# drocheam/optrace

Measured on AMD Instinct MI355X. Metric: ray-surface-intersections/s, higher is better.
Workload: dtype f64

## Files before the change

optrace_amd/csrc/ot_api.hip:

```cpp
#include <cstdlib>
#include <cstring>
#include <string>

#include "ot_host.hpp"
#include "ot_selftest.hpp"

static thread_local std::string g_err;

int fail(int code, const std::string& msg) {
    g_err = msg;
    return code;
}

extern "C" int ot_abi_version(void) { return OT_ABI_VERSION; }
extern "C" const char* ot_last_error(void) { return g_err.c_str(); }
extern "C" int ot_device_count(void) {
    int n = 0;
    if (hipGetDeviceCount(&n) != hipSuccess) return OT_ERR_NO_DEVICE;
    return n;
}

int require_device() {
    int n = 0;
    if (hipGetDeviceCount(&n) != hipSuccess || n <= 0)
        return fail(OT_ERR_NO_DEVICE, "no HIP device available; this library has no CPU fallback");
    return OT_OK;
}

static void* ws_alloc(size_t bytes) {
    void* p = nullptr;
    if (hipMalloc(&p, bytes) != hipSuccess || !p) {
        (void)hipGetLastError();
        return nullptr;
    }
    return p;
}
static void ws_release(void* p) { (void)hipFree(p); }
static void ws_sync() { (void)hipDeviceSynchronize(); }
static ot_scratch::Pool& scratch_pool() {
    static ot_scratch::Pool pool({ws_alloc, ws_release, ws_sync}, [] {
        const char* v = std::getenv("OT_SCRATCH_CAP_GB");
        const double gb = v ? std::atof(v) : 64.0;
        return (size_t)((gb > 0.0 ? gb : 64.0) * 1e9);
    }());
    return pool;
}

ot_scratch::Lease workspace(int purpose, size_t bytes, hipStream_t st) {
    int dev = 0;
    if (hipGetDevice(&dev) != hipSuccess) return {};
    return ot_scratch::Lease(scratch_pool(), dev, purpose, (void*)st, bytes);
}

extern "C" int ot_scratch_trim(void) {
    if (int rc = require_device()) return rc;
    scratch_pool().trim();
    return OT_OK;
}

extern "C" int ot_scratch_set_cap(int64_t bytes) {
    if (bytes < 0) return fail(OT_ERR_INVALID, "ot_scratch_set_cap: negative cap");
    scratch_pool().set_cap((size_t)bytes);
    return OT_OK;
}

extern "C" int ot_scratch_stats(int64_t* kept_bytes, int32_t* blocks, int32_t* leased) {
    size_t kept = 0;
    int nb = 0, busy = 0;
    scratch_pool().stats(&kept, &nb, &busy);
    if (kept_bytes) *kept_bytes = (int64_t)kept;
    if (blocks) *blocks = nb;
    if (leased) *leased = busy;
    return OT_OK;
}

int cu_count() {
    int dev = 0;
    hipDeviceProp_t prop;
    if (hipGetDevice(&dev) == hipSuccess && hipGetDeviceProperties(&prop, dev) == hipSuccess && prop.multiProcessorCount > 0)
        return prop.multiProcessorCount;
    return 256;
}

extern "C" int ot_selftest_arith(int32_t op, int32_t operand_class, int64_t n, uint64_t seed, int64_t* mismatches,
                                 double* first_bad4, void* stream) {
    if (!mismatches || !first_bad4 || n < 0) return fail(OT_ERR_INVALID, "ot_selftest_arith: bad argument");
    if (op < OT_ST_DIV || op > OT_ST_DIV_SHARED || operand_class < OT_CLS_WIDE || operand_class > OT_CLS_COSINE)
        return fail(OT_ERR_INVALID, "ot_selftest_arith: unknown operation or operand class");
    if (int rc = require_device()) return rc;
    hipStream_t st = (hipStream_t)stream;
    char* scratch = nullptr;
    HIP_TRY(hipMalloc((void**)&scratch, 64));
    hipError_t e = hipMemsetAsync(scratch, 0, 64, st);
    unsigned long long host[2] = {0, 0};
    double bad[4] = {0, 0, 0, 0};
    if (e == hipSuccess && n > 0) {
        hipLaunchKernelGGL(selftest_arith_kernel, dim3((unsigned)(cu_count() * 8)), dim3(256), 0, st, (int)op,
                           (int)operand_class, n, seed, (unsigned long long*)scratch, (double*)(scratch + 16));
        e = hipGetLastError();
    }
    if (e == hipSuccess) e = hipMemcpyAsync(host, scratch, 16, hipMemcpyDeviceToHost, st);
    if (e == hipSuccess) e = hipMemcpyAsync(bad, scratch + 16, 32, hipMemcpyDeviceToHost, st);
    if (e == hipSuccess) e = hipStreamSynchronize(st);
    (void)hipFree(scratch);
    HIP_TRY(e);
    *mismatches = (int64_t)host[0];
    std::memcpy(first_bad4, bad, sizeof(bad));
    return OT_OK;
}

extern "C" int ot_selftest_eval(int32_t op, int64_t n, const double* a, const double* b, const double* c, double* core_out,
                                double* ieee_out, void* stream) {
    if (n < 0 || (n && (!a || !core_out || !ieee_out))) return fail(OT_ERR_INVALID, "ot_selftest_eval: bad argument");
    if (op < OT_ST_DIV || op > OT_ST_DIV_SHARED) return fail(OT_ERR_INVALID, "ot_selftest_eval: unknown operation");
    if (int rc = require_device()) return rc;
    if (n == 0) return OT_OK;
    hipLaunchKernelGGL(selftest_eval_kernel, grid_for(n), dim3(256), 0, (hipStream_t)stream, (int)op, n, a, b, c, core_out,
                       ieee_out);
    HIP_TRY(hipGetLastError());
    return OT_OK;
}
```

optrace_amd/csrc/ot_device.hpp:

```cpp
#pragma once
#include <hip/hip_runtime.h>
#include <math.h>

#include "ot_scene.hpp"

#define OT_DEV __device__ __forceinline__
#define OT_HD __host__ __device__ __forceinline__

#define OT_CONST __attribute__((address_space(4)))
template <class T>
OT_DEV const OT_CONST T* as_const(const T* p) {
    return (const OT_CONST T*)p;
}

struct V3 {
    double x, y, z;
};

OT_DEV double dot3(const V3& a, const V3& b) { return a.x * b.x + a.y * b.y + a.z * b.z; }

OT_DEV V3 cross3(const V3& a, const V3& b) {
    V3 n;
    n.x = a.y * b.z - a.z * b.y;
    n.y = a.z * b.x - a.x * b.z;
    n.z = a.x * b.y - a.y * b.x;
    return n;
}

OT_DEV double ot_sqrt(double x) {
    double y = __builtin_amdgcn_rsq(x);
    double g = x * y;
    double h = 0.5 * y;
    double r = __builtin_fma(-h, g, 0.5);
    g = __builtin_fma(g, r, g);
    h = __builtin_fma(h, r, h);
    double d = __builtin_fma(-g, g, x);
    g = __builtin_fma(d, h, g);
    d = __builtin_fma(-g, g, x);
    g = __builtin_fma(d, h, g);
    return (x == 0.0 || x == __builtin_inf()) ? x : g;
}

OT_DEV double ot_rcp3(double d) {
    double r = __builtin_amdgcn_rcp(d);
    r = __builtin_fma(__builtin_fma(-d, r, 1.0), r, r);
    return __builtin_fma(__builtin_fma(-d, r, 1.0), r, r);
}

OT_DEV double ot_div_r(double n, double d, double r) {
    double q = n * r;
    return __builtin_fma(__builtin_fma(-d, q, n), r, q);
}

OT_DEV double ot_rsqrt(double x) {
    double y = __builtin_amdgcn_rsq(x);
    double e = __builtin_fma(-(x * y), y, 1.0);
    y = __builtin_fma(0.5 * y, e, y);
    e = __builtin_fma(-(x * y), y, 1.0);
    return __builtin_fma(0.5 * y, e, y);
}

OT_DEV V3 normalize3(const V3& a) {
    const double l = ot_sqrt(a.x * a.x + a.y * a.y + a.z * a.z);
    const double il = ot_rcp3(l);
    V3 r = {ot_div_r(a.x, l, il), ot_div_r(a.y, l, il), ot_div_r(a.z, l, il)};
    return r;
}

OT_HD double ot_div(double n, double d) {
#if defined(__HIP_DEVICE_COMPILE__)
    return ot_div_r(n, d, ot_rcp3(d));
#else
    return n / d;
#endif
}

OT_DEV V3 along(const V3& p, const V3& s, double t) {
    V3 r = {p.x + s.x * t, p.y + s.y * t, p.z + s.z * t};
    return r;
}

#include "ot_spline.hpp"

#define OT_HIT_CLOSED 0
#define OT_HIT_ILLINOIS 1
#define OT_HIT_SPLINE 2

template <class SF>
OT_HD double data_values_rel(SF& sf, double x, double y, PatchCache* pc = nullptr) {
    const double* t = sf.tab;
    const int n = sf.nk;
    double v;
    const UniformKnots ukv = {sf.ku_t0, sf.ku_h, sf.ku_inv_h, sf.ku_lo, sf.ku_hi,
                              (sf.ku_h > 0.0) ? OT_SPL_K + 1 : (1 << 30), n - OT_SPL_K - 2};
    const UniformKnots* const uk = &ukv;
    if (sf.kind == OT_SURF_DATA1D) {
        v = spl1_eval<OT_SPL_K>(t, n, t + n, sf.inv_h, hypot(x, y), uk, pc);
    } else {
        double xr = x, yr = y;
        if (sf.rot) {
            xr = x * sf.cna - y * sf.sna;
            yr = x * sf.sna + y * sf.cna;
        }
        v = spl2_eval<OT_SPL_K, OT_SPL_K>(t, n, t, n, t + n, sf.inv_h, xr, sf.sgn * yr, pc, uk);
    }
    return sf.sgn * (v - sf.offs);
}

template <class SF>
OT_HD void data_gradient(SF& sf, double x, double y, double& gx, double& gy, PatchCache* pc = nullptr) {
    const double* t = sf.tab;
    const int n = sf.nk;
    const UniformKnots ukv = {sf.ku_t0, sf.ku_h, sf.ku_inv_h, sf.ku_lo, sf.ku_hi,
                              (sf.ku_h > 0.0) ? OT_SPL_K + 1 : (1 << 30), n - OT_SPL_K - 2};
    const UniformKnots* const uk = &ukv;
    if (sf.kind == OT_SURF_DATA1D) {
        const double r = hypot(x, y);
        double d1;
        if (!spl1_grad_cached(t + n, r, uk, pc, d1)) d1 = spl1_eval<OT_SPL_K - 1>(t, n, t + 2 * n, sf.inv_h, r, uk);
        const double nr = sf.sgn * d1;
        const double rr = sqrt(x * x + y * y);
        gx = nr * ((rr > 0.0) ? x / rr : 1.0);
        gy = nr * ((rr > 0.0) ? y / rr : 0.0);
        return;
    }
    double xr = x, yr = y;
    if (sf.rot && !sf.deriv_unrot) {
        xr = x * sf.cna - y * sf.sna;
        yr = x * sf.sna + y * sf.cna;
    }
    const int nc = (n - OT_SPL_K - 1), ncx = (n - OT_SPL_K - 2) * nc;
    const double* c = t + n;
    double nxn, nyn;
    if (spl2_grad_cached(t, n, c, sf.inv_h, xr, sf.sgn * yr, pc, nxn, nyn, uk)) {
        nxn = nxn * sf.sgn;
    } else {
        nxn = spl2_eval<OT_SPL_K - 1, OT_SPL_K>(t + 1, n - 2, t, n, c + nc * nc, sf.inv_h, xr, sf.sgn * yr) * sf.sgn;
        nyn = spl2_eval<OT_SPL_K, OT_SPL_K - 1>(t, n, t + 1, n - 2, c + nc * nc + ncx, sf.inv_h, xr, sf.sgn * yr);
    }
    if (sf.rot) {
        gx = nxn * sf.cpa - nyn * sf.spa;
        gy = nxn * sf.spa + nyn * sf.cpa;
    } else {
        gx = nxn;
        gy = nyn;
    }
}

template <class SF>
OT_HD bool mask_table(SF& sf, double dx, double dy) {
    const uint32_t* words = (const uint32_t*)(sf.tab + sf.mask_off);
    const int n = sf.mask_n;
    int64_t cell;
    if (sf.kind == OT_SURF_DATA1D) {
        const int i = (int)(sqrt(dx * dx + dy * dy) * sf.mask_scale);
        cell = i < n ? i : n - 1;
    } else {
        double xr = dx, yr = dy;
        if (sf.rot) {
            xr = dx * sf.cna - dy * sf.sna;
            yr = dx * sf.sna + dy * sf.cna;
        }
        yr = sf.sgn * yr;
        int ix = (int)floor((xr + sf.mask_r) * sf.mask_scale), iy = (int)floor((yr + sf.mask_r) * sf.mask_scale);
        ix = ix < 0 ? 0 : (ix < n ? ix : n - 1);
        iy = iy < 0 ? 0 : (iy < n ? iy : n - 1);
        cell = (int64_t)iy * n + ix;
    }
    return (words[cell >> 5] >> (uint32_t)(cell & 31)) & 1u;
}

template <bool TABLES = true, class SF>
OT_DEV bool surf_mask(SF& sf, double x, double y) {
    if (sf.kind == OT_SURF_RECT || sf.kind == OT_SURF_SLIT) {
        double dx = x - sf.px, dy = y - sf.py;
        double xr = dx, yr = dy;
        if (sf.rot) {
            xr = dx * sf.cna - dy * sf.sna;
            yr = dx * sf.sna + dy * sf.cna;
        }
        bool outer = (sf.ox_lo <= xr) && (xr <= sf.ox_hi) && (sf.oy_lo <= yr) && (yr <= sf.oy_hi);
        if (sf.kind == OT_SURF_RECT) return outer;
        bool inner = (sf.ix_lo <= xr) && (xr <= sf.ix_hi) && (sf.iy_lo <= yr) && (yr <= sf.iy_hi);
        return outer && !inner;
    }
    double dx = x - sf.px, dy = y - sf.py;
    double r2 = dx * dx + dy * dy;
    bool in = r2 <= sf.r_eps2;
    if (sf.kind == OT_SURF_RING) in = in && (sf.ri_eps2 <= r2);
    if (TABLES && (sf.kind == OT_SURF_DATA1D || sf.kind == OT_SURF_DATA2D) && sf.mask_n) {
        if (in) in = mask_table(sf, dx, dy);
    }
    return in;
}

template <class SF>
OT_DEV double asph_poly(SF& sf, double r) {
    double y = 0.0;
    for (int j = sf.ncoeff - 1; j >= 0; j--) {
        y = y * r + sf.coeff[j];
        y = y * r + 0.0;
    }
    y = y * r + 0.0;
    return y;
}

template <class SF>
OT_DEV double asph_poly_deriv(SF& sf, double r) {
    double y = 0.0;
    for (int j = sf.ncoeff - 1; j >= 0; j--) {
        y = y * r + sf.dcoeff[j];
        y = y * r + 0.0;
    }
    return y;
}

#define OT_ASPH_CHUNK 4
OT_HD int asph_padded(int ncoeff) { return (ncoeff + OT_ASPH_CHUNK - 1) / OT_ASPH_CHUNK * OT_ASPH_CHUNK; }

template <bool DERIV, class SF>
OT_DEV double asph_poly_long(SF& sf, double r) {
    const int npad = asph_padded(sf.ncoeff);
    const OT_CONST double* c = (const OT_CONST double*)sf.tab + (DERIV ? npad : 0);
    double y = 0.0;
#pragma unroll 1
    for (int j = npad - OT_ASPH_CHUNK; j >= 0; j -= OT_ASPH_CHUNK) {
        const double c0 = c[j], c1 = c[j + 1], c2 = c[j + 2], c3 = c[j + 3];
        y = (y * r + c3) * r;
        y = (y * r + c2) * r;
        y = (y * r + c1) * r;
        y = (y * r + c0) * r;
    }
    return y;
}

template <int LEVEL = OT_HIT_SPLINE, class SF>
OT_DEV double surf_values_rel(SF& sf, double x, double y, PatchCache* pc = nullptr) {
    if (sf.kind == OT_SURF_TILTED) return x * sf.mx + y * sf.my;
    if (LEVEL >= OT_HIT_SPLINE && (sf.kind == OT_SURF_DATA1D || sf.kind == OT_SURF_DATA2D)) return data_values_rel(sf, x, y, pc);
    if (sf.kind == OT_SURF_CONIC) {
        double r2 = x * x + y * y;
        return ot_div(sf.rho * r2, 1 + sqrt(1 - sf.k1rho2 * r2));
    }
    double r = sqrt(x * x + y * y);
    double rr = r * r;
    double z = ot_div(sf.rho * rr, 1 + sqrt(1 - sf.k1rho2 * rr));
    if (LEVEL >= OT_HIT_SPLINE && sf.ncoeff > OT_MAX_ASPH)
        z += asph_poly_long<false>(sf, r) * r;
    else
        z += asph_poly(sf, r);
    return z;
}

template <int LEVEL = OT_HIT_SPLINE, class SF>
OT_DEV double surf_values(SF& sf, double x, double y, PatchCache* pc = nullptr) {
    if (sf.flat) return sf.z_max;
    if (surf_mask<(LEVEL >= OT_HIT_SPLINE)>(sf, x, y)) return sf.pz + surf_values_rel<LEVEL>(sf, x - sf.px, y - sf.py, pc);
    if (sf.kind == OT_SURF_TILTED || (LEVEL >= OT_HIT_SPLINE && sf.kind == OT_SURF_DATA2D)) {
        double dx = x - sf.px, dy = y - sf.py;
        double rr = sqrt(dx * dx + dy * dy);
        double c = (rr > 0.0) ? dx / rr : 1.0, sn = (rr > 0.0) ? dy / rr : 0.0;
        return sf.pz + surf_values_rel<LEVEL>(sf, sf.r_edge * c, sf.r_edge * sn, pc);
    }
    return sf.edge_val;
}

template <bool INSIDE = false, int LEVEL = OT_HIT_SPLINE, class SF>
OT_DEV V3 surf_normal(SF& sf, double x, double y, PatchCache* pc = nullptr) {
    constexpr bool TABLES = LEVEL >= OT_HIT_SPLINE;
    V3 n = {0.0, 0.0, 1.0};
    if (sf.kind < OT_SURF_CONIC) return n;
    if (LEVEL == OT_HIT_CLOSED && sf.kind != OT_SURF_CONIC) return n;
    if (sf.kind == OT_SURF_TILTED) {
        if (!INSIDE && !surf_mask<TABLES>(sf, x, y)) return n;
        V3 m = {sf.nx, sf.ny, sf.nz};
        return m;
    }
    if (sf.flat) return n;
    if (!INSIDE && !surf_mask<TABLES>(sf, x, y)) return n;
    double dx = x - sf.px, dy = y - sf.py;
    if (sf.kind == OT_SURF_DATA1D || sf.kind == OT_SURF_DATA2D) {
        if (LEVEL < OT_HIT_SPLINE) return n;
        double gx, gy;
        data_gradient(sf, dx, dy, gx, gy, pc);
        V3 m = {-gx, -gy, 1.0};
        return normalize3(m);
    }
    if (sf.kind == OT_SURF_CONIC) {
        if (sf.k == 0.0) {
            n.x = sf.nrho * dx;
            n.y = sf.nrho * dy;
            n.z = ot_sqrt(1 - sf.rho2 * (dx * dx) - sf.rho2 * (dy * dy));
            return n;
        }
        const double r2 = dx * dx + dy * dy;
        const double q = ot_sqrt(1 - sf.krho2 * r2);
        const double iq = ot_rcp3(q);
        n.x = ot_div_r(sf.nrho * dx, q, iq);
        n.y = ot_div_r(sf.nrho * dy, q, iq);
        n.z = ot_sqrt(1 - (n.x * n.x + n.y * n.y));
        return n;
    }
    double rm = ot_sqrt(dx * dx + dy * dy);
    double fr = ot_div(rm * sf.rho, ot_sqrt(1 - sf.k1rho2 * (rm * rm)));
    if (LEVEL >= OT_HIT_SPLINE && sf.ncoeff > OT_MAX_ASPH)
        fr += asph_poly_long<true>(sf, rm);
    else
        fr += asph_poly_deriv(sf, rm);
    const double irm = ot_rcp3(rm);
    double c = (rm > 0.0) ? ot_div_r(dx, rm, irm) : 1.0;
    double s = (rm > 0.0) ? ot_div_r(dy, rm, irm) : 0.0;
    V3 m = {-(fr * c), -(fr * s), 1.0};
    return normalize3(m);
}

template <class SF>
OT_DEV void handle_abnormal_f(SF& sf, const V3& p, const V3& s, V3& ph, bool& hit, double f);
template <int LEVEL = OT_HIT_SPLINE, class SF>
OT_DEV void handle_abnormal(SF& sf, const V3& p, const V3& s, V3& ph, bool& hit, PatchCache* pc = nullptr) {
    double zs = surf_values<LEVEL>(sf, ph.x, ph.y, pc);
    handle_abnormal_f(sf, p, s, ph, hit, ph.z - zs);
}

template <class SF>
OT_DEV void handle_abnormal_f(SF& sf, const V3& p, const V3& s, V3& ph, bool& hit, double f) {
    bool dev = fabs(f) > OT_C_EPS;
    bool beh = p.z > sf.z_beh;
    bool neg = ph.z < p.z - OT_C_EPS;
    if ((neg || dev) && !beh) {
        double tnm = (sf.z_max - p.z) / s.z;
        ph = along(p, s, tnm);
        hit = false;
    }
    if (beh) {
        ph = p;
        hit = false;
    }
}

template <class SF>
OT_DEV void find_hit_conic_form(SF& sf, const bool sphere, const bool plain, const V3& p, const V3& s, V3& ph, bool& hit) {
    double ox = p.x - sf.px, oy = p.y - sf.py, oz = p.z - sf.pz;
    double ozk = oz * sf.k1;
    double B = s.x * ox + s.y * oy + s.z * (ozk - sf.inv_rho);
    double C = oy * oy + ox * ox + oz * (ozk - sf.two_inv_rho);
    double A = 1.0, D, t1, t2;
    if (plain) {
        D = ot_sqrt(B * B - C);
        t1 = -B - D;
        t2 = -B + D;
    } else {
        if (!sphere) A = 1 + sf.k * (s.z * s.z);
        D = ot_sqrt(B * B - C * A);
        const bool bp = B >= 0;
        const double q = -(B + (bp ? D : -D));
// ... 496 lines not shown
```

optrace_amd/csrc/ot_selftest.hpp:

```cpp
#pragma once
#include "ot_device.hpp"

#define OT_ST_DIV 0
#define OT_ST_SQRT 1
#define OT_ST_NORMALIZE 2
#define OT_ST_DIV_SHARED 3

#define OT_CLS_WIDE 0
#define OT_CLS_GEOMETRY 1
#define OT_CLS_INDEX 2
#define OT_CLS_COSINE 3

OT_DEV double st_make(uint64_t bits, int e_lo, int e_hi, bool sign_rnd) {
    const uint64_t mant = bits & 0xfffffffffffffull;
    const uint32_t r = (uint32_t)(bits >> 52);
    const int span = e_hi - e_lo + 1;
    const int e = e_lo + (int)((r & 0x7ffu) * (uint32_t)span >> 11);
    const uint64_t sign = sign_rnd ? ((uint64_t)(r >> 11) & 1ull) << 63 : 0ull;
    const uint64_t u = sign | ((uint64_t)(e + 1023) << 52) | mant;
    return __longlong_as_double((long long)u);
}

OT_DEV double st_operand(uint64_t bits, int cls, int op) {
    switch (cls) {
        case OT_CLS_WIDE:
            if (op == OT_ST_SQRT) return st_make(bits, -760, 1020, false);
            if (op == OT_ST_NORMALIZE) return st_make(bits, -250, 250, true);
            return st_make(bits, -500, 500, true);
        case OT_CLS_GEOMETRY: return st_make(bits, -20, 14, op != OT_ST_SQRT);
        case OT_CLS_INDEX: {
            const double u = (double)(bits >> 11) * 0x1.0p-53;
            return 1.0 + 1.5 * u;
        }
        default: {
            const double m = st_make(bits, 0, 0, false);
            const int k = (int)((bits >> 52) & 0x3f);
            const double small = ldexp(m, -(k < 61 ? k : 60));
            return ((bits >> 58) & 1) ? 1.0 - 0.5 * small : small;
        }
    }
}

OT_DEV bool st_same(double a, double b) {
    return __double_as_longlong(a) == __double_as_longlong(b) || (a != a && b != b);
}

OT_DEV int st_eval(int op, double a, double b, double c, double* core, double* ieee) {
    switch (op) {
        case OT_ST_DIV:
            core[0] = ot_div(a, b);
            ieee[0] = a / b;
            return 1;
        case OT_ST_SQRT:
            core[0] = ot_sqrt(fabs(a));
            ieee[0] = sqrt(fabs(a));
            return 1;
        case OT_ST_NORMALIZE: {
            const V3 v = {a, b, c};
            const V3 n = normalize3(v);
            const double l = sqrt(a * a + b * b + c * c);
            core[0] = n.x, core[1] = n.y, core[2] = n.z;
            ieee[0] = a / l, ieee[1] = b / l, ieee[2] = c / l;
            return 3;
        }
        default: {
            const double r = ot_rcp3(c);
            core[0] = ot_div_r(a, c, r), core[1] = ot_div_r(b, c, r);
            ieee[0] = a / c, ieee[1] = b / c;
            return 2;
        }
    }
}

__global__ __launch_bounds__(256) void selftest_arith_kernel(int op, int cls, int64_t n, uint64_t seed,
                                                             unsigned long long* __restrict__ out, double* __restrict__ bad) {
    unsigned long long mism = 0;
    const int64_t stride = (int64_t)gridDim.x * blockDim.x;
    for (int64_t i = (int64_t)blockIdx.x * blockDim.x + threadIdx.x; i < n; i += stride) {
        Philox p = philox4x32((uint32_t)i, (uint32_t)(i >> 32), 0x53454c46u, (uint32_t)op, (uint32_t)seed, (uint32_t)(seed >> 32));
        const uint64_t w0 = ((uint64_t)p.c[1] << 32) | p.c[0], w1 = ((uint64_t)p.c[3] << 32) | p.c[2];
        double a = st_operand(w0, cls, op), b = st_operand(w1, cls, op), c = 1.0;
        if (op >= OT_ST_NORMALIZE) {
            Philox q = philox4x32((uint32_t)i, (uint32_t)(i >> 32), 0x53454c47u, (uint32_t)op, (uint32_t)seed, (uint32_t)(seed >> 32));
            c = st_operand(((uint64_t)q.c[1] << 32) | q.c[0], cls, op);
        }
        double core[3], ieee[3];
        const int k = st_eval(op, a, b, c, core, ieee);
        bool ok = true;
        for (int j = 0; j < k; j++) ok = ok && st_same(core[j], ieee[j]);
        if (!ok) {
            if (mism == 0 && atomicAdd(&out[1], 1ull) == 0ull) {
                bad[0] = a, bad[1] = b, bad[2] = c, bad[3] = core[0];
            }
            mism++;
        }
    }
#pragma unroll
    for (int o = 32; o > 0; o >>= 1) mism += __shfl_xor(mism, o);
    if ((threadIdx.x & 63) == 0 && mism) atomicAdd(&out[0], mism);
}

__global__ __launch_bounds__(256) void selftest_eval_kernel(int op, int64_t n, const double* __restrict__ a,
                                                            const double* __restrict__ b, const double* __restrict__ c,
                                                            double* __restrict__ core_out, double* __restrict__ ieee_out) {
    const int64_t i = (int64_t)blockIdx.x * blockDim.x + threadIdx.x;
    if (i >= n) return;
    double core[3] = {0, 0, 0}, ieee[3] = {0, 0, 0};
    st_eval(op, a[i], b ? b[i] : 1.0, c ? c[i] : 1.0, core, ieee);
    for (int j = 0; j < 3; j++) {
        core_out[i + j * n] = core[j];
        ieee_out[i + j * n] = ieee[j];
    }
}
```

optrace_amd/csrc/ot_trace.hpp:

```cpp
#pragma once
#include "ot_device.hpp"
#include "ot_generate.hpp"

OT_DEV void count_event(unsigned int* cnt, int nt, int info, int sec, bool cond) {
    unsigned long long m = __ballot(cond);
    if (m != 0ull) {
        int lane = __lane_id();
        if (lane == (int)__ffsll((long long)m) - 1) atomicAdd(&cnt[info * nt + sec], (unsigned int)__popcll(m));
    }
}

struct RayState {
    V3 p, s;
    float w, wl;
    float polx, poly, polz;
    double n_cur;
};

template <bool POL>
OT_DEV void compute_polarization(const V3& s, const V3& s_, const RayState& r, float& npx, float& npy, float& npz,
                                 double& A_ts, double& A_tp) {
#pragma clang fp contract(fast)
    const double inv_sqrt2 = 0.7071067811865475;
    if (!POL) {
        A_ts = inv_sqrt2;
        A_tp = inv_sqrt2;
        return;
    }
    bool mask = (s.x != s_.x) || (s.y != s_.y) || (s.z != s_.z);
    V3 ps = cross3(s_, s);
    const double l2 = ps.x * ps.x + ps.y * ps.y + ps.z * ps.z;
    double inv = rsqrt(l2);
    ps.x *= inv;
    ps.y *= inv;
    ps.z *= inv;
    V3 pp = cross3(ps, s);
    V3 pol = {(double)r.polx, (double)r.poly, (double)r.polz};
    A_ts = dot3(ps, pol);
    A_tp = dot3(pp, pol);
    if (!mask) {
        A_ts = inv_sqrt2;
        A_tp = inv_sqrt2;
    }
    V3 pp_ = cross3(ps, s_);
    if (mask) {
        npx = (float)(ps.x * A_ts + pp_.x * A_tp);
        npy = (float)(ps.y * A_ts + pp_.y * A_tp);
        npz = (float)(ps.z * A_ts + pp_.z * A_tp);
    }
    const bool small = mask && l2 < 0x1p-40;
    if (__ballot(small) != 0ull) {
        if (small) {
            const double sp = dot3(s_, pol);
            npx = (float)(pol.x - s.x * sp);
            npy = (float)(pol.y - s.y * sp);
            npz = (float)(pol.z - s.z * sp);
        }
    }
}

OT_DEV double fast_rcp(double x) {
    double y = __builtin_amdgcn_rcp(x);
    y = fma(fma(-x, y, 1.0), y, y);
    y = fma(fma(-x, y, 1.0), y, y);
    return y;
}

#ifndef OT_POL_NEAR
#define OT_POL_NEAR 0x1p-52
#endif

OT_DEV bool refraction_polarization(const V3& n, const V3& s, const V3& s_, double ns, const RayState& r, double& A,
                                    double& B, double& M, double& tp, double& sp) {
    const V3 pol = {(double)r.polx, (double)r.poly, (double)r.polz};
    sp = __builtin_fma(s.z, pol.z, __builtin_fma(s.y, pol.y, s.x * pol.x));
    const double np_ = __builtin_fma(n.z, pol.z, __builtin_fma(n.y, pol.y, n.x * pol.x));
    const double P = __builtin_fma(-sp, sp, __builtin_fma(pol.z, pol.z, __builtin_fma(pol.y, pol.y, pol.x * pol.x)));
    tp = __builtin_fma(ns, sp, -np_);
    const V3 e = {__builtin_fma(-ns, s.x, n.x), __builtin_fma(-ns, s.y, n.y), __builtin_fma(-ns, s.z, n.z)};
    M = __builtin_fma(e.z, e.z, __builtin_fma(e.y, e.y, e.x * e.x));
    A = P * M;
    B = tp * tp;
    bool mask = (s.x != s_.x) || (s.y != s_.y) || (s.z != s_.z);
    const bool near = !(M >= OT_POL_NEAR);
    const unsigned long long moved = __ballot(s.x != s_.x) | __ballot(s.y != s_.y) | __ballot(s.z != s_.z);
    if (__ballot(near) != 0ull || moved != __ballot(true)) {
        if (near || !mask) {
            const V3 m = cross3(n, s);
            double half = 0.5 * P;
            if (!mask || !(dot3(m, m) > 0)) {
                mask = false;
                half = 0.5;
            }
            A = 2 * half;
            B = half;
            M = 1;
            tp = 0;
        }
    }
    return mask;
}

OT_DEV void same_medium_polarization(const V3& s, const V3& s_, const RayState& r, float& npx, float& npy, float& npz,
                                     double& A_ts2, double& A_tp2) {
    const bool mask = (s.x != s_.x) || (s.y != s_.y) || (s.z != s_.z);
    A_ts2 = 0.5;
    A_tp2 = 0.5;
    if (mask) {
        const V3 ps = normalize3(cross3(s_, s));
        const V3 pp = cross3(ps, s);
        const V3 pol = {(double)r.polx, (double)r.poly, (double)r.polz};
        const double A_ts = dot3(ps, pol), A_tp = dot3(pp, pol);
        const V3 pp_ = cross3(ps, s_);
        npx = (float)(ps.x * A_ts + pp_.x * A_tp);
        npy = (float)(ps.y * A_ts + pp_.y * A_tp);
        npz = (float)(ps.z * A_ts + pp_.z * A_tp);
        A_ts2 = A_ts * A_ts;
        A_tp2 = A_tp * A_tp;
    }
}

template <bool POL>
OT_DEV bool refract(const V3& n, RayState& r, float& wn, float& npx, float& npy, float& npz, double N) {
    V3 s = r.s;
    double ns = dot3(n, s);
    double W = ot_sqrt(1 - N * N * (1 - ns * ns));
    double Nns = N * ns;
    double q = Nns - W;
    V3 s_ = {s.x * N - n.x * q, s.y * N - n.y * q, s.z * N - n.z * q};

    double A = 1, B = 0.5, M = 1, tp, sp;
    bool bend = false;
    if (POL) {
        if (N == 1.0) {
            double A_ts2, A_tp2;
            same_medium_polarization(s, s_, r, npx, npy, npz, A_ts2, A_tp2);
            A = A_ts2 + A_tp2;
            B = A_tp2;
        } else {
            bend = refraction_polarization(n, s, s_, ns, r, A, B, M, tp, sp);
        }
    }
    const double d1 = Nns + W, d2 = __builtin_fma(N, W, ns), den = d1 * d2;
    const double d2s = d2 * d2, den2 = den * den;
    const double rr = fast_rcp(M * den2);
    double T = 4 * (Nns * W) * (__builtin_fma(A, d2s, B * __builtin_fma(d1, d1, -d2s)) * rr);
    if (Nns == 0) T = __builtin_nan("");
    if (POL && bend) {
        const double k = tp * (rr * den2);
        const double g = k * (1 - __builtin_fma(-q, ns, N)), h = __builtin_fma(k, W - ns, -sp);
        asm("" : "+v"(npx), "+v"(npy), "+v"(npz));
        npx = (float)__builtin_fma(g, n.x, __builtin_fma(h, s.x, (double)npx));
        npy = (float)__builtin_fma(g, n.y, __builtin_fma(h, s.y, (double)npy));
        npz = (float)__builtin_fma(g, n.z, __builtin_fma(h, s.z, (double)npz));
    }
    const bool tir = !isfinite(W);
    if (tir) T = 0;
    wn = (float)((double)r.w * T);
    r.s = s_;
    return tir;
}

template <bool POL, class SF, class EL>
OT_DEV void refract_ideal(SF& sf, EL& el, RayState& r, const V3& pn, float& npx, float& npy,
                          float& npz) {
    V3 s0 = r.s;
    double fsz = el.f / s0.z;
    V3 s = {s0.x * fsz - (pn.x - sf.px), s0.y * fsz - (pn.y - sf.py), el.f};
    s = normalize3(s);
    s.x = s.x * el.fsign;
    s.y = s.y * el.fsign;
    s.z = s.z * el.fsign;
    r.s = s;
    double A_ts, A_tp;
    compute_polarization<POL>(s0, s, r, npx, npy, npz, A_ts, A_tp);
}

template <class OL>
OT_DEV bool outline_clip(OL o, const V3& p, const V3& s, V3& pn, float& wn) {
    bool inside = (o[0] < pn.x) && (pn.x < o[1]) && (o[2] < pn.y) && (pn.y < o[3]) && (o[4] < pn.z) && (pn.z < o[5]);
    if (inside) return false;
    double t = __builtin_nan("");
    double T;
    T = (o[0] - p.x) / s.x; if (T > 0 && !(t <= T)) t = T;
    T = (o[1] - p.x) / s.x; if (T > 0 && !(t <= T)) t = T;
    T = (o[2] - p.y) / s.y; if (T > 0 && !(t <= T)) t = T;
    T = (o[3] - p.y) / s.y; if (T > 0 && !(t <= T)) t = T;
    T = (o[4] - p.z) / s.z; if (T > 0 && !(t <= T)) t = T;
    T = (o[5] - p.z) / s.z; if (T > 0 && !(t <= T)) t = T;
    pn = along(p, s, t);
    wn = 0.f;
    return true;
}

template <bool POL, class SC, class SF>
OT_DEV bool hurb_bend(SC& sc, SF& sf, RayState& r, const V3& pn, float& wn, float& npx,
                      float& npy, float& npz, bool hwnh, double za, double zb) {
    double a_, b_;
    V3 b;
    bool inside;
    hurb_props(sf, pn.x, pn.y, a_, b_, b, inside);
    bool bend = hwnh && inside;
    V3 a = {-b.y, b.x, b.z};
    V3 s = r.s;
    double sa_ = dot3(s, a), sb_ = dot3(s, b);
    double cos_psi_a = ot_sqrt(1 - sa_ * sa_);
    double cos_psi_b = ot_sqrt(1 - sb_ * sb_);
    float wlm = r.wl * (float)1e-9;
    double k = ot_div(2 * M_PI * r.n_cur, (double)wlm);
    double tan_sig_b = ot_div(sc.hurb_factor, 2 * b_ * cos_psi_b * 1e-3 * k);
    double tan_sig_a = ot_div(sc.hurb_factor, 2 * a_ * cos_psi_a * 1e-3 * k);
    double tan_tha = fabs(tan_sig_a) * za;
    double tan_thb = fabs(tan_sig_b) * zb;
    V3 sa = normalize3(cross3(b, s));
    V3 sb = cross3(s, sa);
    V3 sab = {s.x + sa.x * tan_tha + sb.x * tan_thb, s.y + sa.y * tan_tha + sb.y * tan_thb,
              s.z + sa.z * tan_tha + sb.z * tan_thb};
    V3 s0 = s;
    if (bend) {
        s = normalize3(sab);
        r.s = s;
    }
    bool neg = s.z < 0;
    if (neg) wn = 0.f;
    if (bend) {
        double A_ts, A_tp;
        compute_polarization<POL>(s0, s, r, npx, npy, npz, A_ts, A_tp);
    }
    return neg;
}

#ifndef OT_STORE_HINT
#define OT_STORE_HINT " sc0 sc1 nt"
#endif
#ifndef OT_STORE_CLOBBER
#define OT_STORE_CLOBBER : "memory"
#endif
OT_DEV void store_f64(const void* base, uint32_t off, double v) {
    const void* b;
    asm volatile("s_mov_b64 %0, %3\n\tglobal_store_dwordx2 %1, %2, %0" OT_STORE_HINT : "=&s"(b) : "v"(off), "v"(v), "s"(base) OT_STORE_CLOBBER);
}
OT_DEV void store_f32(const void* base, uint32_t off, float v) {
    const void* b;
    asm volatile("s_mov_b64 %0, %3\n\tglobal_store_dword %1, %2, %0" OT_STORE_HINT : "=&s"(b) : "v"(off), "v"(v), "s"(base) OT_STORE_CLOBBER);
}

template <bool POL>
OT_DEV void store_section(const ot_rays& R, uint32_t o8, uint32_t o4, int sec, bool pw, const V3& p, float w, double n,
                          float px, float py, float pz) {
    const int64_t N = R.N;
    const int64_t nt = R.nt;
    if (pw) {
        store_f64(R.p + N * sec, o8, p.x);
        store_f64(R.p + N * (sec + nt), o8, p.y);
        store_f64(R.p + N * (sec + 2 * nt), o8, p.z);
        store_f32(R.w + N * sec, o4, w);
    }
    if (R.n) store_f64(R.n + N * sec, o8, n);
    if (POL && R.pol) {
        store_f32(R.pol + N * sec, o4, px);
        store_f32(R.pol + N * (sec + nt), o4, py);
        store_f32(R.pol + N * (sec + 2 * nt), o4, pz);
    }
}

struct PlaneBases {
    const double *px, *py, *pz, *n;
    const float *w, *qx, *qy, *qz;
    int64_t N;
};
template <bool POL>
OT_DEV PlaneBases plane_bases(const ot_rays& R) {
    const int64_t N = R.N, nt = R.nt;
    PlaneBases b = {R.p, R.p + N * nt, R.p + N * 2 * nt, R.n, R.w, nullptr, nullptr, nullptr, N};
    if (POL && R.pol) {
        b.qx = R.pol;
        b.qy = R.pol + N * nt;
        b.qz = R.pol + N * 2 * nt;
    }
    return b;
}
OT_DEV void store_pol_next(PlaneBases& b, uint32_t o4, float px, float py, float pz) {
    store_f32(b.qx, o4, px);
    store_f32(b.qy, o4, py);
    store_f32(b.qz, o4, pz);
    b.qx += b.N, b.qy += b.N, b.qz += b.N;
}
template <bool POL>
OT_DEV void store_section_next(PlaneBases& b, uint32_t o8, uint32_t o4, bool pw, const V3& p, float w, double n, float px,
                               float py, float pz) {
    if (pw) {
        store_f64(b.px, o8, p.x);
        store_f64(b.py, o8, p.y);
        store_f64(b.pz, o8, p.z);
        store_f32(b.w, o4, w);
    }
    if (b.n) {
        store_f64(b.n, o8, n);
        b.n += b.N;
    }
    b.px += b.N, b.py += b.N, b.pz += b.N, b.w += b.N;
    if (POL && b.qx) store_pol_next(b, o4, px, py, pz);
}
#ifndef OT_RUNNING_BASES
#define OT_RUNNING_BASES 1
#endif

struct TailState {
    V3 p;
    float w;
};
#define OT_STORE_ALL 0
#define OT_STORE_NONE 1
#define OT_STORE_POL 2
template <bool POL, int SPEC, int FEAT, int STORE = OT_STORE_ALL, class SC>
OT_DEV bool trace_ray(SC& sc, const ot_rays& R, uint32_t local, uint64_t ray, RayState& r,
                      const double* __restrict__ hurb_normals, uint64_t seed, unsigned int* msgs, const double* ltab,
                      int lj, double* patch_lds, TailState* tail = nullptr, int sec_first = 0,
                      int sec_end = 0x7fffffff) {
    constexpr bool TAB = (SPEC == 1);
    constexpr bool TAIL = (STORE == OT_STORE_NONE);
    constexpr bool ALL = (STORE == OT_STORE_ALL);
    constexpr bool POL_ONLY = (STORE == OT_STORE_POL);
    constexpr bool FULL = (FEAT & 1) != 0;
    constexpr int LEVEL = FEAT / 2;
    constexpr bool IDEAL_FILTER = FULL || LEVEL >= OT_HIT_ILLINOIS;
    constexpr bool NUMERIC = LEVEL >= OT_HIT_ILLINOIS;
    constexpr bool SPLINE = LEVEL >= OT_HIT_SPLINE;
    const double* lrow = ltab + OT_MAX_LINES + lj;
    const uint32_t o8 = local * 8u, o4 = local * 4u;
    PatchCache pcache = {patch_lds + threadIdx.x, 256, nullptr};
    PatchCache* const pc = SPLINE ? &pcache : nullptr;
    const int nt = sc.nt;
    const auto surfaces = as_const(sc.surfaces);
    const auto hot = as_const(sc.hot);
    const auto media = as_const(sc.media);
    const auto filters = as_const(sc.filters);
    const auto pool = as_const(sc.pool);
    bool ok = true;
    r.n_cur = (SPEC == 2) ? lrow[(3 * sc.n_steps) * OT_MAX_LINES] : medium_n<TAB>(media[sc.n0], pool, r.wl);
#if OT_RUNNING_BASES
    PlaneBases planes = {};
    if (!TAIL) planes = plane_bases<POL>(R);
    if (ALL)
        store_section_next<POL>(planes, o8, o4, sec_first <= 0 && 0 < sec_end, r.p, r.w, r.n_cur, r.polx, r.poly, r.polz);
    if (POL_ONLY) store_pol_next(planes, o4, r.polx, r.poly, r.polz);
#else
    if (ALL)
        store_section<POL>(R, o8, o4, 0, sec_first <= 0 && 0 < sec_end, r.p, r.w, r.n_cur, r.polx, r.poly, r.polz);
#endif

    for (int i = 0; i < sc.n_steps; i++) {
        auto& st = hot[i];
        const int form = st.form;
        if (TAIL && i + 1 == sc.n_steps) {
            tail->p = r.p;
            tail->w = r.w;
        }
        auto& sf = surfaces[st.surf];
        const int kind = st.kind;
        V3 pn = r.p;
        float wn = r.w;
        float npx = r.polx, npy = r.poly, npz = r.polz;
        const bool hw = r.w > 0;
        V3 ph;
        bool hit = false, ill = false;
        if (SPLINE) {
            pcache.key = nullptr;
        }
        if (hw) {
            if (form != OT_HOT_OTHER)
                find_hit_hot(st, form, r.p, r.s, ph, hit);
            else
                ok &= find_hit<LEVEL>(sf, r.p, r.s, ph, hit, ill, pc);
            pn = ph;
        }
        if (NUMERIC) count_event(msgs, nt, OT_INFO_ILL_COND, i + 1, hw && ill);
        const bool hwh = hw && hit, hwnh = hw && !hit;
        bool tir = false, neg = false, clip = false;
        double n_next = r.n_cur;

        if (kind <= OT_STEP_IDEAL) {
            if (hwnh) {
                wn = 0.f;
                if (kind == OT_STEP_LENS_BACK) pn = r.p;
            }
            double Nq;
            if (SPEC == 2) {
                n_next = lrow[(3 * i + 0) * OT_MAX_LINES];
                Nq = lrow[(3 * i + 1) * OT_MAX_LINES];
            } else {
                n_next = medium_n<TAB>(media[st.n_next], pool, r.wl);
                Nq = ot_div(r.n_cur, n_next);
            }
            if (hwh) {
                if (IDEAL_FILTER && kind == OT_STEP_IDEAL) {
                    refract_ideal<POL>(st, st, r, pn, npx, npy, npz);
                } else {
                    V3 n;
                    if (form != OT_HOT_OTHER)
                        n = hot_normal(st, form, pn.x, pn.y);
                    else
                        n = surf_normal<true, LEVEL>(sf, pn.x, pn.y, pc);
                    tir = refract<POL>(n, r, wn, npx, npy, npz, Nq);
                }
            }
        } else if (IDEAL_FILTER && kind == OT_STEP_FILTER) {
            if (hwh) {
                double T = (SPEC == 2) ? lrow[(3 * i + 2) * OT_MAX_LINES] : filter_T<TAB>(filters[st.filter], pool, r.wl);
                wn = (float)((double)r.w * T);
            }
        } else {
            if (hwh) wn = 0.f;
            if (FULL && st.hurb) {
                double za, zb;
                if (TAB && hurb_normals) {
                    za = (hurb_normals + (2 * (int64_t)st.hurb_slot + 0) * R.N)[ray];
                    zb = (hurb_normals + (2 * (int64_t)st.hurb_slot + 1) * R.N)[ray];
                } else {
                    philox_normal2(seed, ray, 0x48555242u, (uint32_t)st.hurb_slot, za, zb);
                }
                neg = hurb_bend<POL>(sc, sf, r, pn, wn, npx, npy, npz, hwnh, za, zb);
            }
            if (FULL) count_event(msgs, nt, OT_INFO_HURB_NEG_DIR, i + 1, neg);
        }
        if (hwnh) clip = outline_clip(sc.outline, r.p, r.s, pn, wn);
        if (__ballot(hwnh || tir) != 0ull) {
            if (kind <= OT_STEP_IDEAL) {
                count_event(msgs, nt, OT_INFO_ABSORB_MISSING, i + 1, hwnh);
                count_event(msgs, nt, OT_INFO_TIR, i, tir);
            }
            count_event(msgs, nt, OT_INFO_OUTLINE_INTERSECTION, i, clip);
        }

        r.p = pn;
        r.w = wn;
        r.polx = npx;
        r.poly = npy;
        r.polz = npz;
        r.n_cur = n_next;
#ifdef OT_NO_SECTION_STORES
        if (i + 1 == sc.n_steps)
#endif
        {
#if OT_RUNNING_BASES
            if (ALL)
                store_section_next<POL>(planes, o8, o4, sec_first <= i + 1 && i + 1 < sec_end, r.p, r.w, r.n_cur, r.polx,
                                        r.poly, r.polz);
            if (POL_ONLY) store_pol_next(planes, o4, r.polx, r.poly, r.polz);
#else
            if (ALL)
                store_section<POL>(R, o8, o4, i + 1, sec_first <= i + 1 && i + 1 < sec_end, r.p, r.w, r.n_cur, r.polx,
                                   r.poly, r.polz);
#endif
        }
    }
    if (ALL) {
        const int64_t N = R.N;
        store_f64(R.s, o8, r.s.x);
        store_f64(R.s + N, o8, r.s.y);
        store_f64(R.s + 2 * N, o8, r.s.z);
    }
    return ok;
}
```

Measured before the change: 127.5 billion.

## Compute section store addresses on demand and trim reciprocal to one Newton step

Removes the running per-plane base pointers and instead recomputes store addresses from section index with scalar-register hints, to cut live vector registers across the step loop. Also copies the hot step record head into scalar registers via an asm barrier, and reduces fast_rcp from two Newton iterations to one, adding a selftest kernel that bounds the resulting reciprocal error. Trades some extra scalar address arithmetic and reduced reciprocal precision (about 2^-48 relative) for lower register pressure and fewer FMAs.

Result: faster. 132.7 billion (median of 6 runs) (+4.0%).

```diff
diff --git a/optrace_amd/csrc/ot_api.hip b/optrace_amd/csrc/ot_api.hip
--- a/optrace_amd/csrc/ot_api.hip
+++ b/optrace_amd/csrc/ot_api.hip
@@ -85,7 +85,8 @@
 extern "C" int ot_selftest_arith(int32_t op, int32_t operand_class, int64_t n, uint64_t seed, int64_t* mismatches,
                                  double* first_bad4, void* stream) {
     if (!mismatches || !first_bad4 || n < 0) return fail(OT_ERR_INVALID, "ot_selftest_arith: bad argument");
-    if (op < OT_ST_DIV || op > OT_ST_DIV_SHARED || operand_class < OT_CLS_WIDE || operand_class > OT_CLS_COSINE)
+    if (op < OT_ST_DIV || op > OT_ST_FAST_RCP || operand_class < OT_CLS_WIDE || operand_class > OT_CLS_RECIPROCAL ||
+        (op == OT_ST_FAST_RCP) != (operand_class == OT_CLS_RECIPROCAL))
         return fail(OT_ERR_INVALID, "ot_selftest_arith: unknown operation or operand class");
     if (int rc = require_device()) return rc;
     hipStream_t st = (hipStream_t)stream;
@@ -94,7 +95,11 @@
     hipError_t e = hipMemsetAsync(scratch, 0, 64, st);
     unsigned long long host[2] = {0, 0};
     double bad[4] = {0, 0, 0, 0};
-    if (e == hipSuccess && n > 0) {
+    if (e == hipSuccess && n > 0 && op == OT_ST_FAST_RCP) {
+        hipLaunchKernelGGL(selftest_rcp_kernel, dim3((unsigned)(cu_count() * 8)), dim3(256), 0, st, n, seed,
+                           (unsigned long long*)scratch, (double*)(scratch + 16));
+        e = hipGetLastError();
+    } else if (e == hipSuccess && n > 0) {
         hipLaunchKernelGGL(selftest_arith_kernel, dim3((unsigned)(cu_count() * 8)), dim3(256), 0, st, (int)op,
                            (int)operand_class, n, seed, (unsigned long long*)scratch, (double*)(scratch + 16));
         e = hipGetLastError();
diff --git a/optrace_amd/csrc/ot_device.hpp b/optrace_amd/csrc/ot_device.hpp
--- a/optrace_amd/csrc/ot_device.hpp
+++ b/optrace_amd/csrc/ot_device.hpp
@@ -51,6 +51,17 @@
     double q = n * r;
     return __builtin_fma(__builtin_fma(-d, q, n), r, q);
 }
+
+template <int STEPS>
+OT_DEV double rcp_newton(double x) {
+    double y = __builtin_amdgcn_rcp(x);
+#pragma unroll
+    for (int k = 0; k < STEPS; k++) y = fma(fma(-x, y, 1.0), y, y);
+    return y;
+}
+#define OT_FAST_RCP_STEPS 1
+#define OT_FAST_RCP_BOUND 0x1p-48
+OT_DEV double fast_rcp(double x) { return rcp_newton<OT_FAST_RCP_STEPS>(x); }
 
 OT_DEV double ot_rsqrt(double x) {
     double y = __builtin_amdgcn_rsq(x);
diff --git a/optrace_amd/csrc/ot_selftest.hpp b/optrace_amd/csrc/ot_selftest.hpp
--- a/optrace_amd/csrc/ot_selftest.hpp
+++ b/optrace_amd/csrc/ot_selftest.hpp
@@ -5,11 +5,13 @@
 #define OT_ST_SQRT 1
 #define OT_ST_NORMALIZE 2
 #define OT_ST_DIV_SHARED 3
+#define OT_ST_FAST_RCP 4
 
 #define OT_CLS_WIDE 0
 #define OT_CLS_GEOMETRY 1
 #define OT_CLS_INDEX 2
 #define OT_CLS_COSINE 3
+#define OT_CLS_RECIPROCAL 4
 
 OT_DEV double st_make(uint64_t bits, int e_lo, int e_hi, bool sign_rnd) {
     const uint64_t mant = bits & 0xfffffffffffffull;
@@ -28,6 +30,7 @@
             if (op == OT_ST_NORMALIZE) return st_make(bits, -250, 250, true);
             return st_make(bits, -500, 500, true);
         case OT_CLS_GEOMETRY: return st_make(bits, -20, 14, op != OT_ST_SQRT);
+        case OT_CLS_RECIPROCAL: return st_make(bits, -60, 60, false);
         case OT_CLS_INDEX: {
             const double u = (double)(bits >> 11) * 0x1.0p-53;
             return 1.0 + 1.5 * u;
@@ -72,6 +75,34 @@
     }
 }
 
+OT_DEV void st_max(double* slot, double v) { atomicMax((unsigned long long*)slot, (unsigned long long)__double_as_longlong(v)); }
+
+__global__ __launch_bounds__(256) void selftest_rcp_kernel(int64_t n, uint64_t seed, unsigned long long* __restrict__ out,
+                                                           double* __restrict__ bad) {
+    unsigned long long over = 0;
+    double e0 = 0.0, e1 = 0.0, e2 = 0.0, e3 = 0.0;
+    const int64_t stride = (int64_t)gridDim.x * blockDim.x;
+    for (int64_t i = (int64_t)blockIdx.x * blockDim.x + threadIdx.x; i < n; i += stride) {
+        Philox p = philox4x32((uint32_t)i, (uint32_t)(i >> 32), 0x53454c46u, (uint32_t)OT_ST_FAST_RCP, (uint32_t)seed,
+                              (uint32_t)(seed >> 32));
+        const double x = st_operand(((uint64_t)p.c[1] << 32) | p.c[0], OT_CLS_RECIPROCAL, OT_ST_FAST_RCP);
+        const double d0 = fabs(fma(-x, rcp_newton<0>(x), 1.0)), d1 = fabs(fma(-x, rcp_newton<1>(x), 1.0));
+        const double d2 = fabs(fma(-x, rcp_newton<2>(x), 1.0)), d3 = fabs(fma(-x, fast_rcp(x), 1.0));
+        e0 = fmax(e0, d0);
+        e1 = fmax(e1, d1);
+        e2 = fmax(e2, d2);
+        e3 = fmax(e3, d3);
+        if (!(d3 <= OT_FAST_RCP_BOUND)) over++;
+    }
+    st_max(&bad[0], e0);
+    st_max(&bad[1], e1);
+    st_max(&bad[2], e2);
+    st_max(&bad[3], e3);
+#pragma unroll
+    for (int o = 32; o > 0; o >>= 1) over += __shfl_xor(over, o);
+    if ((threadIdx.x & 63) == 0 && over) atomicAdd(&out[0], over);
+}
+
 __global__ __launch_bounds__(256) void selftest_arith_kernel(int op, int cls, int64_t n, uint64_t seed,
                                                              unsigned long long* __restrict__ out, double* __restrict__ bad) {
     unsigned long long mism = 0;
diff --git a/optrace_amd/csrc/ot_trace.hpp b/optrace_amd/csrc/ot_trace.hpp
--- a/optrace_amd/csrc/ot_trace.hpp
+++ b/optrace_amd/csrc/ot_trace.hpp
@@ -57,13 +57,6 @@
             npz = (float)(pol.z - s.z * sp);
         }
     }
-}
-
-OT_DEV double fast_rcp(double x) {
-    double y = __builtin_amdgcn_rcp(x);
-    y = fma(fma(-x, y, 1.0), y, y);
-    y = fma(fma(-x, y, 1.0), y, y);
-    return y;
 }
 
 #ifndef OT_POL_NEAR
@@ -245,66 +238,54 @@
     asm volatile("s_mov_b64 %0, %3\n\tglobal_store_dword %1, %2, %0" OT_STORE_HINT : "=&s"(b) : "v"(off), "v"(v), "s"(base) OT_STORE_CLOBBER);
 }
 
+OT_DEV uint32_t on_demand(int sec) {
+    asm("" : "+s"(sec));
+    return (uint32_t)sec;
+}
+
+OT_DEV void store_pol(const ot_rays& R, uint32_t o4, int sec, float px, float py, float pz) {
+    const uint64_t N = (uint64_t)R.N, first = N * on_demand(sec), plane = N * on_demand(R.nt);
+    store_f32(R.pol + first, o4, px);
+    store_f32(R.pol + (first + plane), o4, py);
+    store_f32(R.pol + (first + 2 * plane), o4, pz);
+}
 template <bool POL>
 OT_DEV void store_section(const ot_rays& R, uint32_t o8, uint32_t o4, int sec, bool pw, const V3& p, float w, double n,
                           float px, float py, float pz) {
-    const int64_t N = R.N;
-    const int64_t nt = R.nt;
     if (pw) {
-        store_f64(R.p + N * sec, o8, p.x);
-        store_f64(R.p + N * (sec + nt), o8, p.y);
-        store_f64(R.p + N * (sec + 2 * nt), o8, p.z);
-        store_f32(R.w + N * sec, o4, w);
-    }
-    if (R.n) store_f64(R.n + N * sec, o8, n);
-    if (POL && R.pol) {
-        store_f32(R.pol + N * sec, o4, px);
-        store_f32(R.pol + N * (sec + nt), o4, py);
-        store_f32(R.pol + N * (sec + 2 * nt), o4, pz);
-    }
-}
-
-struct PlaneBases {
-    const double *px, *py, *pz, *n;
-    const float *w, *qx, *qy, *qz;
-    int64_t N;
+        const uint64_t N = (uint64_t)R.N, first = N * on_demand(sec), plane = N * on_demand(R.nt);
+        store_f64(R.p + first, o8, p.x);
+        store_f64(R.p + (first + plane), o8, p.y);
+        store_f64(R.p + (first + 2 * plane), o8, p.z);
+        store_f32(R.w + first, o4, w);
+    }
+    if (R.n) store_f64(R.n + (uint64_t)R.N * on_demand(sec), o8, n);
+    if (POL && R.pol) store_pol(R, o4, sec, px, py, pz);
+}
+
+struct HotHeadValues {
+    int32_t kind, form, surf, n_next, filter, hurb, hurb_slot;
+    double px, py, pz, r_eps2, z_max, z_lo, z_hi, k1, inv_rho, two_inv_rho;
 };
-template <bool POL>
-OT_DEV PlaneBases plane_bases(const ot_rays& R) {
-    const int64_t N = R.N, nt = R.nt;
-    PlaneBases b = {R.p, R.p + N * nt, R.p + N * 2 * nt, R.n, R.w, nullptr, nullptr, nullptr, N};
-    if (POL && R.pol) {
-        b.qx = R.pol;
-        b.qy = R.pol + N * nt;
-        b.qz = R.pol + N * 2 * nt;
-    }
-    return b;
-}
-OT_DEV void store_pol_next(PlaneBases& b, uint32_t o4, float px, float py, float pz) {
-    store_f32(b.qx, o4, px);
-    store_f32(b.qy, o4, py);
-    store_f32(b.qz, o4, pz);
-    b.qx += b.N, b.qy += b.N, b.qz += b.N;
-}
-template <bool POL>
-OT_DEV void store_section_next(PlaneBases& b, uint32_t o8, uint32_t o4, bool pw, const V3& p, float w, double n, float px,
-                               float py, float pz) {
-    if (pw) {
-        store_f64(b.px, o8, p.x);
-        store_f64(b.py, o8, p.y);
-        store_f64(b.pz, o8, p.z);
-        store_f32(b.w, o4, w);
-    }
-    if (b.n) {
-        store_f64(b.n, o8, n);
-        b.n += b.N;
-    }
-    b.px += b.N, b.py += b.N, b.pz += b.N, b.w += b.N;
-    if (POL && b.qx) store_pol_next(b, o4, px, py, pz);
-}
-#ifndef OT_RUNNING_BASES
-#define OT_RUNNING_BASES 1
-#endif
+template <class REC>
+struct HotHead : HotHeadValues {
+    decltype((((REC*)nullptr)->k)) k;
+    decltype((((REC*)nullptr)->ri_eps2)) ri_eps2;
+    decltype((((REC*)nullptr)->nrho)) nrho;
+    decltype((((REC*)nullptr)->rho2)) rho2;
+    decltype((((REC*)nullptr)->krho2)) krho2;
+    decltype((((REC*)nullptr)->f)) f;
+    decltype((((REC*)nullptr)->fsign)) fsign;
+};
+template <class REC>
+OT_DEV HotHeadValues hot_head_values(REC& h) {
+    return {h.kind, h.form, h.surf, h.n_next, h.filter, h.hurb, h.hurb_slot, h.px, h.py, h.pz, h.r_eps2, h.z_max, h.z_lo,
+            h.z_hi, h.k1, h.inv_rho, h.two_inv_rho};
+}
+template <class REC>
+OT_DEV HotHead<REC> hot_head(const HotHeadValues& v, REC& h) {
+    return {v, h.k, h.ri_eps2, h.nrho, h.rho2, h.krho2, h.f, h.fsign};
+}
 
 struct TailState {
     V3 p;
@@ -339,19 +320,13 @@
     const auto pool = as_const(sc.pool);
     bool ok = true;
     r.n_cur = (SPEC == 2) ? lrow[(3 * sc.n_steps) * OT_MAX_LINES] : medium_n<TAB>(media[sc.n0], pool, r.wl);
-#if OT_RUNNING_BASES
-    PlaneBases planes = {};
-    if (!TAIL) planes = plane_bases<POL>(R);
-    if (ALL)
-        store_section_next<POL>(planes, o8, o4, sec_first <= 0 && 0 < sec_end, r.p, r.w, r.n_cur, r.polx, r.poly, r.polz);
-    if (POL_ONLY) store_pol_next(planes, o4, r.polx, r.poly, r.polz);
-#else
-    if (ALL)
-        store_section<POL>(R, o8, o4, 0, sec_first <= 0 && 0 < sec_end, r.p, r.w, r.n_cur, r.polx, r.poly, r.polz);
-#endif
+    if (ALL) store_section<POL>(R, o8, o4, 0, sec_first <= 0 && 0 < sec_end, r.p, r.w, r.n_cur, r.polx, r.poly, r.polz);
+    if (POL_ONLY) store_pol(R, o4, 0, r.polx, r.poly, r.polz);
 
     for (int i = 0; i < sc.n_steps; i++) {
-        auto& st = hot[i];
+        auto head = hot_head_values(hot[i]);
+        asm("" : "+s"(head.inv_rho), "+s"(head.two_inv_rho));
+        const auto st = hot_head(head, hot[i]);
         const int form = st.form;
         if (TAIL && i + 1 == sc.n_steps) {
             tail->p = r.p;
@@ -443,16 +418,10 @@
         if (i + 1 == sc.n_steps)
 #endif
         {
-#if OT_RUNNING_BASES
-            if (ALL)
-                store_section_next<POL>(planes, o8, o4, sec_first <= i + 1 && i + 1 < sec_end, r.p, r.w, r.n_cur, r.polx,
-                                        r.poly, r.polz);
-            if (POL_ONLY) store_pol_next(planes, o4, r.polx, r.poly, r.polz);
-#else
             if (ALL)
                 store_section<POL>(R, o8, o4, i + 1, sec_first <= i + 1 && i + 1 < sec_end, r.p, r.w, r.n_cur, r.polx,
                                    r.poly, r.polz);
-#endif
+            if (POL_ONLY) store_pol(R, o4, i + 1, r.polx, r.poly, r.polz);
         }
     }
     if (ALL) {
```
